# spawner1145/vae-tagger

Hardware: AMD Instinct MI355X
Metric: images/sec encode+tag, 1024^2 bf16 (higher is better)
Workload: dtype bf16

## Files before the change

vae_tagger_amd/csrc/capi.hip:

```cpp
#include <math.h>
#include <string.h>

#include "vt_context.h"
#include "vt_eval.h"

using namespace vt;

namespace {
__global__ void dbg_checksum_kernel(const unsigned int* __restrict__ p, long long n, unsigned long long* __restrict__ out) {
    unsigned long long acc = 0;
    for (long long i = (long long)blockIdx.x * blockDim.x + threadIdx.x; i < n; i += (long long)gridDim.x * blockDim.x) acc += (unsigned long long)p[i] * (unsigned long long)(i % 1021 + 1);
    atomicAdd(out, acc);
}
constexpr int DBG_SLOTS = 256;
}

void vt::dbg_sum(vt_context* c, const void* p, size_t bytes, hipStream_t s) {
    if (!c->dbg_on || !c->dbg || c->dbg_n >= DBG_SLOTS) return;
    hipLaunchKernelGGL(dbg_checksum_kernel, dim3(64), dim3(256), 0, s, (const unsigned int*)p, (long long)(bytes / 4), c->dbg + c->dbg_n);
    ++c->dbg_n;
}

extern "C" {

// ... 125 lines not shown
            d.bn_shift = (const float*)c->upload(sh.data(), H * 4);
            d.bn_w = (const float*)c->upload(g->v.data(), H * 4);
            d.bn_b = (const float*)c->upload(b->v.data(), H * 4);
            d.bn_mean = (const float*)c->upload(m->v.data(), H * 4);
            d.bn_var = (const float*)c->upload(v->v.data(), H * 4);
            if (!d.bn_scale || !d.bn_shift || !d.bn_w || !d.bn_b || !d.bn_mean || !d.bn_var) return c->fail(VT_ERR_HIP, "upload failed for batch norm");
        }
        if (d.use_self) {
            const char* p = "self_attention_post.";
            std::string s(p);
            G((s + "norm.weight").c_str(), H, &d.sa.ln_w); G((s + "norm.bias").c_str(), H, &d.sa.ln_b);
            G((s + "q_proj.weight").c_str(), H * H, &d.sa.q_w); G((s + "q_proj.bias").c_str(), H, &d.sa.q_b);
            G((s + "k_proj.weight").c_str(), H * H, &d.sa.k_w); G((s + "k_proj.bias").c_str(), H, &d.sa.k_b);
            G((s + "v_proj.weight").c_str(), H * H, &d.sa.v_w); G((s + "v_proj.bias").c_str(), H, &d.sa.v_b);
            G((s + "out_proj.weight").c_str(), H * H, &d.sa.o_w); G((s + "out_proj.bias").c_str(), H, &d.sa.o_b);
        }
        if (d.use_cross) {
            G("query_generator.weight", (int64_t)512 * H * 64, &d.qg_w); G("query_generator.bias", 512, &d.qg_b);
            G("cross_attention.q_proj.weight", 256 * 512, &d.cx_q_w); G("cross_attention.q_proj.bias", 256, &d.cx_q_b);
            G("cross_attention.k_proj.weight", 256 * H, &d.cx_k_w); G("cross_attention.k_proj.bias", 256, &d.cx_k_b);
            G("cross_attention.v_proj.weight", 256 * H, &d.cx_v_w); G("cross_attention.v_proj.bias", 256, &d.cx_v_b);
            G("cross_attention.out_proj.weight", 512 * 256, &d.cx_o_w); G("cross_attention.out_proj.bias", 512, &d.cx_o_b);
        }
        const int dims[4] = {H * 64, 1024, 512, 256};
        for (int i = 0; i < 3; ++i) {
            char k[64];
            snprintf(k, sizeof k, "classifier.%d.weight", 4 * i); G(k, (int64_t)dims[i + 1] * dims[i], &d.cls_w[i]);
            snprintf(k, sizeof k, "classifier.%d.bias", 4 * i); G(k, dims[i + 1], &d.cls_b[i]);
            snprintf(k, sizeof k, "classifier.%d.weight", 4 * i + 1); G(k, dims[i + 1], &d.cls_ln_w[i]);
            snprintf(k, sizeof k, "classifier.%d.bias", 4 * i + 1); G(k, dims[i + 1], &d.cls_ln_b[i]);
        }
        G("classifier.12.weight", (int64_t)N * 256, &d.cls_w[3]);
        G("classifier.12.bias", N, &d.cls_b[3]);
    }
#undef G
    for (auto it = c->weights.begin(); it != c->weights.end();)
        it = (it->first.compare(0, 8, "encoder.") != 0 && it->first.compare(0, 8, "decoder.") != 0) ? c->weights.erase(it) : ++it;
    c->dec_finalized = true;
    return VT_OK;
}

size_t vt_decode_workspace_bytes(const vt_context* c, int B, int h, int w) {
    if (!c || !c->dec_configured || B <= 0 || h <= 0 || w <= 0) return 0;
    return align_up(vt_decoder_workspace_floats(B, c->dec.latent_channels, h, w) * 4);
}

int vt_decode_logits(vt_context* c, const float* latent, int B, int h, int w, float* logits, void* ws, size_t ws_bytes,
                     void* stream) {
    if (!c) return VT_ERR_INVALID;
    DeviceGuard guard(c);
    if (!c->dec_finalized) return c->fail(VT_ERR_STATE, "decoder weights not finalized");
    if (!latent || !logits || !ws || B <= 0 || h <= 0 || w <= 0) return c->fail(VT_ERR_INVALID, "vt_decode_logits: bad argument");
    if (ws_bytes < vt_decode_workspace_bytes(c, B, h, w)) return c->fail(VT_ERR_WORKSPACE, "vt_decode_logits: workspace too small");
    HIPCK(c, vt_decoder_forward(c->dec, latent, B, h, w, (float*)ws, logits, (hipStream_t)stream), "decoder_forward");
    return VT_OK;
}

int vt_get_confidence(vt_context* c, const float* logits, int B, int N, float* conf, int64_t* idx, void* stream) {
    if (!c) return VT_ERR_INVALID;
    DeviceGuard guard(c);
    if (!logits || !conf || !idx || B <= 0 || N <= 0) return c->fail(VT_ERR_INVALID, "vt_get_confidence: bad argument");
    HIPCK(c, vt_decoder_sort(logits, B, N, conf, (long long*)idx, (hipStream_t)stream), "decoder_sort");
    return VT_OK;
}

int vt_summarize_confidence(vt_context* c, const float* conf, const int64_t* idx, int B, int N, float threshold, int K,
                            float* top_conf, int32_t* top_idx, float* stats, void* stream) {
    if (!c) return VT_ERR_INVALID;
    DeviceGuard guard(c);
    if (!conf || !idx || !top_conf || !top_idx || !stats || B <= 0 || N <= 0 || K <= 0) return c->fail(VT_ERR_INVALID, "vt_summarize_confidence: bad argument");
    HIPCK(c, vt_decoder_summary(conf, (const long long*)idx, B, N, threshold, K, top_conf, (int*)top_idx, stats, (hipStream_t)stream), "decoder_summary");
    return VT_OK;
}

int vt_summarize_confidence_per_class(vt_context* c, const float* conf, const int64_t* idx, int B, int N, const float* class_thresholds,
                                      int K, float* top_conf, int32_t* top_idx, float* stats, void* stream) {
    if (!c) return VT_ERR_INVALID;
    DeviceGuard guard(c);
    if (!conf || !idx || !class_thresholds || !top_conf || !top_idx || !stats || B <= 0 || N <= 0 || K <= 0)
        return c->fail(VT_ERR_INVALID, "vt_summarize_confidence_per_class: bad argument");
    HIPCK(c, vt_decoder_summary_per_class(conf, (const long long*)idx, B, N, class_thresholds, K, top_conf, (int*)top_idx, stats,
                                          (hipStream_t)stream), "decoder_summary_per_class");
    return VT_OK;
}

int vt_status(vt_context* c, int clear, int* status_out, void* stream) {
    if (!c) return VT_ERR_INVALID;
    DeviceGuard guard(c);
    if (!status_out) return c->fail(VT_ERR_INVALID, "vt_status: null output");
    hipStream_t s = (hipStream_t)stream;
    int v = 0;
    HIPCK(c, hipMemcpyAsync(&v, c->status, sizeof(int), hipMemcpyDeviceToHost, s), "vt_status copy");
    const hipError_t ec = clear ? hipMemsetAsync(c->status, 0, sizeof(int), s) : hipSuccess;
    HIPCK(c, hipStreamSynchronize(s), "vt_status sync");
    HIPCK(c, ec, "vt_status clear");
    *status_out = v;
    return VT_OK;
}

int vt_status_async(vt_context* c, int clear, int* status_out, void* stream) {
    if (!c) return VT_ERR_INVALID;
    DeviceGuard guard(c);
    if (!status_out) return c->fail(VT_ERR_INVALID, "vt_status_async: null output");
    hipStream_t s = (hipStream_t)stream;
    HIPCK(c, hipMemcpyAsync(status_out, c->status, sizeof(int), hipMemcpyDefault, s), "vt_status_async copy");
    if (clear) HIPCK(c, hipMemsetAsync(c->status, 0, sizeof(int), s), "vt_status_async clear");
    return VT_OK;
// ... 162 lines not shown

int vt_eval_merge(vt_context* c, void* dst, size_t dst_bytes, int N, int T, long long dst_capacity, long long dst_n_seen,
                  const vt_eval_source* sources, int W, void* stream) {
    if (!c) return VT_ERR_INVALID;
    DeviceGuard guard(c);
    if (int r = eval_check_state(c, "vt_eval_merge (dst)", dst, dst_bytes, N, T, dst_capacity)) return r;
    if (!sources || W < 1 || W > VT_EVAL_MAX_MERGE) return c->fail(VT_ERR_INVALID, "vt_eval_merge: null sources or W = %d outside [1, %d]", W, VT_EVAL_MAX_MERGE);
    if (dst_n_seen < 0 || dst_n_seen > VT_EVAL_MAX_N_SEEN || (dst_capacity > 0 && dst_n_seen > dst_capacity))
        return c->fail(VT_ERR_INVALID, "vt_eval_merge: dst_n_seen = %lld outside [0, capacity = %lld]", dst_n_seen, dst_capacity);
    const EvalLayout l = vt_eval_layout(N, T, dst_capacity);
    EvalMergeArg a;
    a.W = W;
    long long total = dst_n_seen;
    for (int w = 0; w < W; ++w) {
        const vt_eval_source& s = sources[w];
        if (int r = eval_check_state(c, "vt_eval_merge (source)", s.state, s.state_bytes, N, T, s.capacity)) return r;
        if (s.n_seen < 0 || s.n_seen > VT_EVAL_MAX_N_SEEN || (s.capacity > 0 && s.n_seen > s.capacity))
            return c->fail(VT_ERR_INVALID, "vt_eval_merge: source %d has n_seen = %lld outside [0, capacity = %lld]", w, s.n_seen, s.capacity);
        if (blocks_overlap(dst, l.total, s.state, vt_eval_layout(N, T, s.capacity).total))
            return c->fail(VT_ERR_INVALID, "vt_eval_merge: source %d is dst or overlaps it", w);
        if (dst_capacity > 0 && s.capacity == 0 && s.n_seen > 0)
            return c->fail(VT_ERR_INVALID, "vt_eval_merge: source %d keeps no keys (capacity 0) for its %lld samples, dst does", w, s.n_seen);
        a.src[w] = EvalMergeSrc{(const char*)s.state, s.capacity, s.n_seen, s.n_seen, total};
        total += s.n_seen;
        if (total > VT_EVAL_MAX_N_SEEN) return c->fail(VT_ERR_INVALID, "vt_eval_merge: %lld samples in all, 2^31 or more", total);
    }
    if (dst_capacity > 0 && total > dst_capacity)
        return c->fail(VT_ERR_INVALID, "vt_eval_merge: dst_n_seen + the sources' samples = %lld exceeds the capacity %lld", total, dst_capacity);
    HIPCK(c, vt_eval_launch_merge(dst, l, N, dst_capacity, a, c->eval_merge_vec, (hipStream_t)stream), "eval_merge");
    return VT_OK;
}

int vt_set_flag(vt_context* c, int flag, int value) {
    if (!c) return VT_ERR_INVALID;
    if (flag == 0) { c->use_halo_conv = value != 0; return VT_OK; }
    if (flag == 1) { c->fuse_gn_stats = value != 0; return VT_OK; }
    if (flag == 2) { c->fuse_gn_apply = value != 0; return VT_OK; }
    if (flag == 3) { c->halo_occ2 = value < 0 ? 0 : (value > 4 ? 4 : value); return VT_OK; }
    if (flag == 4) { c->res_fp16 = value != 0; return VT_OK; }
    if (flag == 5) { c->conv_in_mfma = value != 0; return VT_OK; }
    if (flag == 6) { c->gemm_short = value != 0; return VT_OK; }
    if (flag == 8) { c->fuse_shortcut = value != 0; return VT_OK; }
    if (flag == 9) { c->attn_qk_kernel = value != 0; return VT_OK; }
    if (flag == 10) { c->pv_stream = value != 0; return VT_OK; }
    if (flag == 11) { c->fp8 = value != 0; return VT_OK; }
    if (flag == 16) { if ((value & 3) == 3 || value < 0 || value > 7) return c->fail(VT_ERR_INVALID, "vt_set_flag(16): tile shape 0..2 (+4: every layer)"); c->fp8_tile = value; return VT_OK; }
    if (flag == 12) { c->attn_pv_kernel = value != 0; return VT_OK; }
    if (flag == 17) { c->attn_proj_kernel = value != 0; return VT_OK; }
    if (flag == 18) { c->f16_ops = value != 0; return VT_OK; }
    if (flag == 19) { c->s2_planar = value != 0; return VT_OK; }
    if (flag == 21) { c->eval_merge_vec = value != 0; return VT_OK; }
    if (flag == 20) { c->conv_out_halo = value != 0; return VT_OK; }
    if (flag == 22) { c->up2_literal = value != 0; return VT_OK; }
    if (flag == 13) { c->s2_halo = value != 0; return VT_OK; }
    if (flag == 14) { c->attn_fp8 = value != 0; return VT_OK; }
    if (flag == 15) { c->proj_fp8 = value != 0; return VT_OK; }
    if (flag == 7) {
        if (value < 0 || value > 2) return c->fail(VT_ERR_INVALID, "vt_set_flag(7): value %d not in 0..2", value);
        c->attn_mode = value;
        return VT_OK;
    }
    return c->fail(VT_ERR_INVALID, "vt_set_flag: unknown flag %d", flag);
}

int vt_profile_num_configs(void) { return VT_NUM_PROF_SLOTS; }

int vt_preprocess_u8(vt_context* c, const uint8_t* in_hwc, int B, int H, int W, float* out_nchw, void* stream) {
    if (!c) return VT_ERR_INVALID;
    DeviceGuard guard(c);
    HIPCK(c, vt_launch_preprocess_u8(in_hwc, out_nchw, B, H, W, (hipStream_t)stream), "vt_preprocess_u8");
    return VT_OK;
}

namespace {
constexpr int RS_BITS = 32 - 8 - 2;
double rs_filter(int kind, double x) {
    if (kind == 0) {
        if (x < 0.0) x = -x;
        return x < 1.0 ? 1.0 - x : 0.0;
    }
    if (-3.0 <= x && x < 3.0) {
        auto sinc = [](double v) { if (v == 0.0) return 1.0; v *= M_PI; return sin(v) / v; };
        return sinc(x) * sinc(x / 3);
    }
    return 0.0;
}
}
extern "C++" {
namespace vt {
int rs_ksize(int in_size, int out_size, int kind) {
    double fs = (double)in_size / out_size;
    if (fs < 1.0) fs = 1.0;
    return (int)ceil((kind == 0 ? 1.0 : 3.0) * fs) * 2 + 1;
}
void rs_table(int in_size, int out_size, int kind, int* tab) {
    const double scale = (double)in_size / out_size;
    double filterscale = scale < 1.0 ? 1.0 : scale;
    const double support = (kind == 0 ? 1.0 : 3.0) * filterscale, ss = 1.0 / filterscale;
    const int ksize = (int)ceil(support) * 2 + 1;
    std::vector<double> w(ksize);
    for (int xx = 0; xx < out_size; ++xx) {
        const double center = (xx + 0.5) * scale;
        int xmin = (int)(center - support + 0.5);
        if (xmin < 0) xmin = 0;
        int xmax = (int)(center + support + 0.5);
        if (xmax > in_size) xmax = in_size;
// ... 119 lines not shown
```

vae_tagger_amd/csrc/decoder.hip:

```cpp
#include "vt_common.h"
#include "vt_decoder.h"
#include "vt_sort_network.h"

namespace {

__global__ __launch_bounds__(256) void dec_pool_kernel(const float* __restrict__ x, int HW, float* __restrict__ pool) {
    __shared__ float red[4];
    const int c = blockIdx.x, b = blockIdx.y, C = gridDim.x;
    const float* xp = x + ((long long)b * C + c) * HW;
    float s = 0.f, m = -INFINITY;
    for (int i = threadIdx.x; i < HW; i += 256) { const float v = xp[i]; s += v; m = fmaxf(m, v); }
    s = block_sum_256(s, red);
    m = block_max_256(m, red);
    if (threadIdx.x == 0) { pool[(b * C + c) * 2] = s / (float)HW; pool[(b * C + c) * 2 + 1] = m; }
}

__global__ void dec_gate_kernel(const float* __restrict__ pool, const float* __restrict__ w0,
                                const float* __restrict__ w2, int C, int R, float* __restrict__ gate) {
    const int b = blockIdx.x, c = threadIdx.x;
    if (c >= C) return;
    float out = 0.f;
    for (int which = 0; which < 2; ++which) {
        for (int r = 0; r < R; ++r) {
            float h = 0.f;
            for (int i = 0; i < C; ++i) h = fmaf(w0[r * C + i], pool[(b * C + i) * 2 + which], h);
            h = fmaxf(h, 0.f);
            out = fmaf(w2[c * R + r], h, out);
        }
    }
    gate[b * C + c] = vt_sigmoid_accurate(out);
}

__global__ __launch_bounds__(256) void dec_spmap_kernel(const float* __restrict__ x, const float* __restrict__ gate,
                                                        int C, int HW, float* __restrict__ sp) {
    const int b = blockIdx.y;
    const int p = blockIdx.x * 256 + threadIdx.x;
    if (p >= HW) return;
    float s = 0.f, m = -INFINITY;
    for (int c = 0; c < C; ++c) {
        const float v = x[((long long)b * C + c) * HW + p] * gate[b * C + c];
        s += v; m = fmaxf(m, v);
    }
    sp[((long long)b * 2) * HW + p] = s / (float)C;
    sp[((long long)b * 2 + 1) * HW + p] = m;
}

__global__ __launch_bounds__(256) void dec_sgate_kernel(const float* __restrict__ sp, const float* __restrict__ w,
                                                        int H, int W, float* __restrict__ sg) {
    __shared__ float sw[98];
    if (threadIdx.x < 98) sw[threadIdx.x] = w[threadIdx.x];
    __syncthreads();
    const int b = blockIdx.y, HW = H * W;
    const int p = blockIdx.x * 256 + threadIdx.x;
    if (p >= HW) return;
    const int y = p / W, x = p - y * W;
    float acc = 0.f;
    for (int c = 0; c < 2; ++c)
        for (int ky = 0; ky < 7; ++ky) {
            const int iy = y + ky - 3;
            if (iy < 0 || iy >= H) continue;
            for (int kx = 0; kx < 7; ++kx) {
                const int ix = x + kx - 3;
                if (ix < 0 || ix >= W) continue;
                acc = fmaf(sw[(c * 7 + ky) * 7 + kx], sp[((long long)b * 2 + c) * HW + iy * W + ix], acc);
            }
        }
    sg[(long long)b * HW + p] = vt_sigmoid_accurate(acc);
}

template <int CO>
__global__ __launch_bounds__(256) void dec_compress_kernel(const float* __restrict__ x, const float* __restrict__ gate,
                                                           const float* __restrict__ sg, const float* __restrict__ w,
                                                           const float* __restrict__ bias,
                                                           const float* __restrict__ bn_scale,
                                                           const float* __restrict__ bn_shift, int C, int H, int W,
                                                           float* __restrict__ pooled) {
    extern __shared__ float smw[];
    __shared__ float red[4];
    __shared__ float sgate[64];
    const int cell = blockIdx.x, b = blockIdx.y, HW = H * W;
    const int cy = cell >> 3, cx = cell & 7;
    for (int i = threadIdx.x; i < CO * C * 9; i += 256) smw[i] = w[i];
    if (threadIdx.x < C) sgate[threadIdx.x] = gate ? gate[b * C + threadIdx.x] : 1.f;
    __syncthreads();
    const int y0 = (cy * H) / 8, y1 = ((cy + 1) * H + 7) / 8;
    const int x0 = (cx * W) / 8, x1 = ((cx + 1) * W + 7) / 8;
    const int ch = y1 - y0, cw = x1 - x0, n = ch * cw;
    float acc[CO];
#pragma unroll
    for (int o = 0; o < CO; ++o) acc[o] = 0.f;
    for (int i = threadIdx.x; i < n; i += 256) {
        const int y = y0 + i / cw, xx = x0 + i % cw;
        float v[CO];
#pragma unroll
        for (int o = 0; o < CO; ++o) v[o] = bias[o];
        for (int ky = 0; ky < 3; ++ky) {
            const int iy = y + ky - 1;
            if (iy < 0 || iy >= H) continue;
            for (int kx = 0; kx < 3; ++kx) {
                const int ix = xx + kx - 1;
                if (ix < 0 || ix >= W) continue;
                const int q = iy * W + ix;
                const float sgv = sg ? sg[(long long)b * HW + q] : 1.f;
                for (int c = 0; c < C; ++c) {
                    const float in = (x[((long long)b * C + c) * HW + q] * sgate[c]) * sgv;
#pragma unroll
                    for (int o = 0; o < CO; ++o) v[o] = fmaf(smw[(o * C + c) * 9 + ky * 3 + kx], in, v[o]);
                }
            }
        }
#pragma unroll
        for (int o = 0; o < CO; ++o) acc[o] += fmaxf(fmaf(v[o], bn_scale[o], bn_shift[o]), 0.f);
    }
#pragma unroll
    for (int o = 0; o < CO; ++o) {
        const float s = block_sum_256(acc[o], red);
        if (threadIdx.x == 0) pooled[((long long)b * CO + o) * 64 + cell] = s / (float)n;
    }
}

// ... 72 lines not shown
    }
#pragma unroll
    for (int o = 0; o < E; ++o) {
        float a = wts.o_b[o];
    #pragma unroll
    for (int e = 0; e < E; ++e) a = fmaf(wts.o_w[o * E + e], att[e], a);
        t[((long long)b * E + o) * 64 + tok] = a + xin[o];
    }
}

#pragma clang diagnostic pop

constexpr int LIN_BT = 8;
__global__ __launch_bounds__(256) void dec_linear_kernel(const float* __restrict__ x, const float* __restrict__ w,
                                                         const float* __restrict__ bias, float* __restrict__ y,
                                                         int B, int IN, int OUT) {
    const int lane = threadIdx.x & 63;
    const int o = blockIdx.x * 4 + (threadIdx.x >> 6);
    if (o >= OUT) return;
    const float* wr = w + (long long)o * IN;
    for (int b0 = 0; b0 < B; b0 += LIN_BT) {
        float acc[LIN_BT];
#pragma unroll
        for (int i = 0; i < LIN_BT; ++i) acc[i] = 0.f;
        for (int k = lane; k < IN; k += 64) {
            const float wv = wr[k];
#pragma unroll
            for (int i = 0; i < LIN_BT; ++i)
                if (b0 + i < B) acc[i] = fmaf(wv, x[(long long)(b0 + i) * IN + k], acc[i]);
        }
#pragma unroll
        for (int i = 0; i < LIN_BT; ++i) {
            const float s = wave_sum(acc[i]);
            if (lane == 0 && b0 + i < B) y[(long long)(b0 + i) * OUT + o] = s + bias[o];
        }
    }
}

__global__ __launch_bounds__(256) void dec_ln_act_kernel(float* __restrict__ y, const float* __restrict__ g,
                                                         const float* __restrict__ bta, int N, int act) {
    __shared__ float red[4];
    float* r = y + (long long)blockIdx.x * N;
    float s = 0.f;
    for (int i = threadIdx.x; i < N; i += 256) s += r[i];
    const float mean = block_sum_256(s, red) / (float)N;
    float v = 0.f;
    for (int i = threadIdx.x; i < N; i += 256) { const float d = r[i] - mean; v = fmaf(d, d, v); }
    const float var = block_sum_256(v, red) / (float)N;
    const float rstd = 1.0f / sqrtf(var + 1e-5f);
    for (int i = threadIdx.x; i < N; i += 256) {
        float t = (r[i] - mean) * rstd * g[i] + bta[i];
        t = act == 0 ? fmaxf(t, 0.f) : (t > 0.f ? t : 0.2f * t);
        r[i] = t;
    }
}

__global__ __launch_bounds__(256) void dec_add_rowmean_kernel(float* __restrict__ flat, const float* __restrict__ att,
                                                              int NF, int NA) {
    __shared__ float red[4];
    const int b = blockIdx.x;
    float s = 0.f;
    for (int i = threadIdx.x; i < NA; i += 256) s += att[(long long)b * NA + i];
    const float m = block_sum_256(s, red) / (float)NA;
    for (int i = threadIdx.x; i < NF; i += 256) flat[(long long)b * NF + i] += m;
}

__global__ __launch_bounds__(64) void dec_cross_attn_kernel(const float* __restrict__ qv, const float* __restrict__ feat,
                                                            const float* __restrict__ k_w, const float* __restrict__ k_b,
                                                            const float* __restrict__ v_w, const float* __restrict__ v_b,
                                                            int CH, int E, int heads, float* __restrict__ out) {
    __shared__ float so[256];
    const int b = blockIdx.x, j = threadIdx.x;
    float f[16];
    for (int c = 0; c < CH; ++c) f[c] = feat[((long long)b * CH + c) * 64 + j];
    const int hd = E / heads;
    const float scale = 1.0f / sqrtf((float)hd);
    for (int h = 0; h < heads; ++h) {
        float s = 0.f;
        for (int d = 0; d < hd; ++d) {
            const int e = h * hd + d;
            float kk = k_b[e];
            for (int c = 0; c < CH; ++c) kk = fmaf(k_w[e * CH + c], f[c], kk);
            s = fmaf(qv[(long long)b * E + e], kk, s);
        }
        s *= scale;
        const float m = wave_max(s);
        const float p = expf(s - m);
        const float den = wave_sum(p);
        for (int d = 0; d < hd; ++d) {
            const int e = h * hd + d;
            float vv = v_b[e];
            for (int c = 0; c < CH; ++c) vv = fmaf(v_w[e * CH + c], f[c], vv);
            const float o = wave_sum(p * vv) / den;
            if (j == 0) so[e] = o;
        }
    }
    __syncthreads();
    for (int e = j; e < E; e += 64) out[(long long)b * E + e] = so[e];
}

__global__ void dec_add_kernel(float* __restrict__ a, const float* __restrict__ b, long long n) {
    const long long i = (long long)blockIdx.x * blockDim.x + threadIdx.x;
    if (i < n) a[i] += b[i];
}

constexpr int SORT_CH = VT_SORT_CH;
// ... 131 lines not shown
    if (tid == 0) {
        float s5 = 0.f;
        for (int i = 0; i < 5 && i < N; ++i) s5 += c[i];
        float* o = stats + (long long)b * 4;
        o[0] = (float)base; o[1] = c[0]; o[2] = s5 / 5.0f; o[3] = (float)s_bad;
    }
}

}

#define CK(e) do { hipError_t _e = (e); if (_e != hipSuccess) return _e; } while (0)
#define CKL() CK(hipGetLastError())

DecHeadShape vt_decoder_head_shape(const DecoderWeights& w) {
    DecHeadShape h;
    const int C = w.latent_channels;
    if (w.plain) { h.hidden = 2; h.dims[0] = C * 16; h.dims[1] = 512; h.dims[2] = 256; h.dims[3] = w.num_classes; h.dims[4] = 0; h.act = 1; }
    else { h.hidden = 3; h.dims[0] = (C / 2) * 64; h.dims[1] = 1024; h.dims[2] = 512; h.dims[3] = 256; h.dims[4] = w.num_classes; h.act = 0; }
    return h;
}

hipError_t vt_dec_linear(const float* x, const float* w, const float* bias, float* y, int B, int IN, int OUT, hipStream_t s) {
    hipLaunchKernelGGL(dec_linear_kernel, dim3((OUT + 3) / 4), dim3(256), 0, s, x, w, bias, y, B, IN, OUT); CKL();
    return hipSuccess;
}
hipError_t vt_dec_ln_act(float* y, const float* g, const float* b, int rows, int N, int act, hipStream_t s) {
    hipLaunchKernelGGL(dec_ln_act_kernel, dim3(rows), dim3(256), 0, s, y, g, b, N, act); CKL();
    return hipSuccess;
}

hipError_t vt_dec_pool(const float* x, int B, int C, int HW, float* pool, hipStream_t s) {
    hipLaunchKernelGGL(dec_pool_kernel, dim3(C, B), dim3(256), 0, s, x, HW, pool); CKL();
    return hipSuccess;
}
hipError_t vt_dec_gate(const float* pool, const float* w0, const float* w2, int B, int C, int R, float* gate, hipStream_t s) {
    hipLaunchKernelGGL(dec_gate_kernel, dim3(B), dim3(64), 0, s, pool, w0, w2, C, R, gate); CKL();
    return hipSuccess;
}
hipError_t vt_dec_sgate(const float* sp, const float* w, int B, int H, int W, float* sg, hipStream_t s) {
    hipLaunchKernelGGL(dec_sgate_kernel, dim3((H * W + 255) / 256, B), dim3(256), 0, s, sp, w, H, W, sg); CKL();
    return hipSuccess;
}

hipError_t vt_dec_cross(const DecoderWeights& w, const float* x, int B, float* cq, float* cqp, float* co, float* cat, float* feat, hipStream_t s) {
    hipLaunchKernelGGL(dec_linear_kernel, dim3(512 / 4), dim3(256), 0, s, x, w.qg_w, w.qg_b, cq, B, 512, 512); CKL();
    hipLaunchKernelGGL(dec_linear_kernel, dim3(256 / 4), dim3(256), 0, s, cq, w.cx_q_w, w.cx_q_b, cqp, B, 512, 256); CKL();
    hipLaunchKernelGGL(dec_cross_attn_kernel, dim3(B), dim3(64), 0, s, cqp, x, w.cx_k_w, w.cx_k_b, w.cx_v_w, w.cx_v_b, 8, 256, w.heads, co); CKL();
    hipLaunchKernelGGL(dec_linear_kernel, dim3(512 / 4), dim3(256), 0, s, co, w.cx_o_w, w.cx_o_b, cat, B, 256, 512); CKL();
    hipLaunchKernelGGL(dec_add_kernel, dim3((B * 512 + 255) / 256), dim3(256), 0, s, cat, cq, (long long)B * 512); CKL();
    hipLaunchKernelGGL(dec_add_rowmean_kernel, dim3(B), dim3(256), 0, s, feat, cat, 512, 512); CKL();
    return hipSuccess;
}

hipError_t vt_decoder_front(const DecoderWeights& w, const float* latent, int B, int H, int Wd, float* ws, float* feat, hipStream_t s) {
    const int C = w.latent_channels, HW = H * Wd;
    if (B <= 0 || H <= 0 || Wd <= 0 || C <= 0 || C > 64) return hipErrorInvalidValue;
    if (w.plain) {
        const int n = C * 16;
        hipLaunchKernelGGL(dec_adaptive_pool_kernel, dim3((n + 255) / 256, B), dim3(256), 0, s, latent, C, H, Wd, 4, 4, feat); CKL();
        return hipSuccess;
    }
    const int CO = C / 2;
    if (CO != 8) return hipErrorInvalidValue;
    float* p = ws;
    float* pool = p; p += (size_t)B * C * 2;
    float* gate = p; p += (size_t)B * C;
    float* sp = p; p += (size_t)B * 2 * HW;
    float* sg = p; p += (size_t)B * HW;
    float* cq = p; p += (size_t)B * 512;
    float* cqp = p; p += (size_t)B * 256;
    float* co = p; p += (size_t)B * 256;
    float* cat = p; p += (size_t)B * 512;
    const float* gptr = nullptr;
    const float* sgptr = nullptr;
    if (w.use_spatial) {
        CK(vt_dec_pool(latent, B, C, HW, pool, s));
        CK(vt_dec_gate(pool, w.ca_w0, w.ca_w2, B, C, w.ca_hidden, gate, s));
        hipLaunchKernelGGL(dec_spmap_kernel, dim3((HW + 255) / 256, B), dim3(256), 0, s, latent, gate, C, HW, sp); CKL();
        CK(vt_dec_sgate(sp, w.sa_w, B, H, Wd, sg, s));
        gptr = gate; sgptr = sg;
    }
    hipLaunchKernelGGL((dec_compress_kernel<8>), dim3(64, B), dim3(256), (size_t)CO * C * 9 * sizeof(float), s, latent, gptr, sgptr,
                       w.fc_w, w.fc_b, w.bn_scale, w.bn_shift, C, H, Wd, feat); CKL();
    if (w.use_self) {
        if (CO % w.heads) return hipErrorInvalidValue;
        if (CO == 8 && w.heads == 8) hipLaunchKernelGGL((dec_self_attn_kernel<8, 8>), dim3(B), dim3(64), 0, s, feat, w.sa, CO, w.heads);
        else hipLaunchKernelGGL((dec_self_attn_kernel<0, 0>), dim3(B), dim3(64), 0, s, feat, w.sa, CO, w.heads);
        CKL();
    }
    if (w.use_cross) CK(vt_dec_cross(w, feat, B, cq, cqp, co, cat, feat, s));
    return hipSuccess;
}

hipError_t vt_decoder_head(const DecHeadShape& h, const DecHeadParams& p, const float* feat, int B, float* hbuf, float* logits, hipStream_t s) {
    const float* x = feat;
    for (int i = 0; i < h.hidden; ++i) {
        CK(vt_dec_linear(x, p.w[i], p.b[i], hbuf, B, h.dims[i], h.dims[i + 1], s));
        CK(vt_dec_ln_act(hbuf, p.ln_w[i], p.ln_b[i], B, h.dims[i + 1], h.act, s));
        x = hbuf; hbuf += (size_t)B * h.dims[i + 1];
    }
    return vt_dec_linear(x, p.w[h.hidden], p.b[h.hidden], logits, B, h.dims[h.hidden], h.dims[h.hidden + 1], s);
}

hipError_t vt_decoder_forward(const DecoderWeights& w, const float* latent, int B, int H, int Wd, float* ws,
                              float* logits, hipStream_t s) {
    const DecHeadShape h = vt_decoder_head_shape(w);
    float* feat = ws;
    float* hbuf = feat + (size_t)B * h.dims[0];
    float* front_ws = hbuf + (size_t)B * (1024 + 512 + 256);
    CK(vt_decoder_front(w, latent, B, H, Wd, front_ws, feat, s));
    DecHeadParams p;
    for (int i = 0; i < 4; ++i) { p.w[i] = w.cls_w[i]; p.b[i] = w.cls_b[i]; }
    for (int i = 0; i < 3; ++i) { p.ln_w[i] = w.cls_ln_w[i]; p.ln_b[i] = w.cls_ln_b[i]; }
    return vt_decoder_head(h, p, feat, B, hbuf, logits, s);
}

size_t vt_decoder_workspace_floats(int B, int C, int H, int Wd) {
    const size_t HW = (size_t)H * Wd;
    return (size_t)B * (C * 2 + C + 2 * HW + HW + (C / 2) * 64 + 1024 + 512 + 256 + 512 + 256 + 256 + 512 + C * 16 + 512 + 256) + 64;
}

hipError_t vt_decoder_sort(const float* logits, int B, int N, float* conf, long long* idx, hipStream_t s) {
    if (N <= 0 || B <= 0) return hipErrorInvalidValue;
    static std::atomic<unsigned long long> attr_done{0};
    CK(vt_once_per_device(attr_done, [&] {
        hipError_t e = hipFuncSetAttribute((const void*)dec_sort_local_kernel<0>, hipFuncAttributeMaxDynamicSharedMemorySize, SORT_CH * 8);
        if (e == hipSuccess) e = hipFuncSetAttribute((const void*)dec_sort_local_kernel<1>, hipFuncAttributeMaxDynamicSharedMemorySize, SORT_CH * 8);
        return e;
    }));
    const int chunks = (N + SORT_CH - 1) / SORT_CH;
    unsigned long long* keys = (unsigned long long*)idx;
    int np = 2;
    while (np < (N < SORT_CH ? N : SORT_CH)) np <<= 1;
    const size_t smem = (size_t)np * 8;
    hipLaunchKernelGGL(dec_sort_local_kernel<0>, dim3(chunks, B), dim3(1024), smem, s, logits, N, keys, conf, idx, chunks == 1 ? 1 : 0); CKL();
    if (chunks == 1) return hipSuccess;
    long long top = SORT_CH;
    while (top < N) top <<= 1;
    const unsigned pair_blocks = (unsigned)((top / 2 + 255) / 256);
    for (long long k = 2LL * SORT_CH; k <= top; k <<= 1) {
        hipLaunchKernelGGL(dec_sort_global_kernel, dim3(pair_blocks, B), dim3(256), 0, s, keys, N, (int)k, 0, 1); CKL();
        for (long long j = k >> 2; j >= SORT_CH; j >>= 1) {
            hipLaunchKernelGGL(dec_sort_global_kernel, dim3(pair_blocks, B), dim3(256), 0, s, keys, N, (int)k, (int)j, 0); CKL();
        }
        hipLaunchKernelGGL(dec_sort_local_kernel<1>, dim3(chunks, B), dim3(1024), (size_t)SORT_CH * 8, s, logits, N, keys, conf, idx, k == top ? 1 : 0); CKL();
    }
    return hipSuccess;
}

hipError_t vt_decoder_summary(const float* conf, const long long* idx, int B, int N, float threshold, int K, float* top_conf,
                              int* top_idx, float* stats, hipStream_t s) {
    if (B <= 0 || N <= 0 || K <= 0) return hipErrorInvalidValue;
    hipLaunchKernelGGL(dec_summary_kernel, dim3(B), dim3(256), 0, s, conf, idx, N, threshold, K, top_conf, top_idx, stats); CKL();
    return hipSuccess;
}

hipError_t vt_decoder_summary_per_class(const float* conf, const long long* idx, int B, int N, const float* class_thresholds, int K,
                                        float* top_conf, int* top_idx, float* stats, hipStream_t s) {
    if (B <= 0 || N <= 0 || K <= 0) return hipErrorInvalidValue;
    hipLaunchKernelGGL(dec_summary_per_class_kernel, dim3(B), dim3(256), 0, s, conf, idx, N, class_thresholds, K, top_conf, top_idx, stats); CKL();
    return hipSuccess;
}
```

vae_tagger_amd/csrc/vt_context.h:

```cpp
#pragma once
#include <hip/hip_runtime.h>
#include <stdarg.h>
#include <stdio.h>

#include <array>
#include <map>
#include <string>
#include <vector>

#include "../../include/vae_tagger_hip.h"
#include "vt_decoder.h"
#include "vt_kernels.h"

namespace vt {

struct HostTensor {
    std::vector<float> v;
    std::vector<int64_t> shape;
    int64_t numel() const { int64_t n = 1; for (auto d : shape) n *= d; return n; }
};

struct ConvW {
    const bf16_t* w = nullptr; const bf16_t* wp = nullptr; const float* b = nullptr; int cin = 0, cout = 0, k = 0;
    const bf16_t* wp2 = nullptr;
// ... 43 lines not shown
    bool has_scaling = false, has_shift = false;
    ConvW conv_in;
    int conv_in_cin() const { return (latent + 31) / 32 * 32; }
    ResnetW mid0, mid1;
    AttnW attn;
    std::vector<UpBlockW> ups;
    NormW norm_out;
    ConvW conv_out;
};

constexpr float FP8_ACT_SCALE = 8.0f;
constexpr float FP8_RES_SCALE = 1.0f;

constexpr size_t ALIGN = 256;
inline size_t align_up(size_t x) { return (x + ALIGN - 1) / ALIGN * ALIGN; }

}

struct vt_context {
    int device = 0;
    std::string err;
    std::map<std::string, vt::HostTensor> weights;
    std::vector<void*> enc_allocs, dec_allocs, imgdec_allocs;
    vt::ImageDecoderW imgdec;
    std::vector<void*>* cur_allocs = &enc_allocs;
    bool pack_fp8 = true;
    void* zeros = nullptr;
    int* status = nullptr;
    vt::EncoderW enc;
    DecoderWeights dec;
    bool dec_configured = false, dec_finalized = false;
    int use_halo_conv = 1;
    int fuse_gn_stats = 1;
    int fuse_gn_apply = 0;
    int res_fp16 = 1;
    int attn_mode = 0;
    int fuse_shortcut = 1;
    int pv_stream = 1;
    int attn_qk_kernel = 1;
    int attn_pv_kernel = 1;
    int fp8 = 0;
    int halo_occ2 = 3;
    int gemm_short = 1;
    int proj_fp8 = 1;
    int attn_fp8 = 1;
    unsigned long long* dbg = nullptr; int dbg_n = 0; bool dbg_on = false;
    int conv_out_halo = 1;
    int s2_planar = 1;
    int eval_merge_vec = 1;
    int f16_ops = 0;
    int attn_proj_kernel = 1;
    int fp8_tile = 0;
    int up2_literal = 0;
    int s2_halo = 1;
    int* rs_host = nullptr; size_t rs_host_ints = 0; hipEvent_t rs_event = nullptr;
    struct RsRingSlot { void* host = nullptr; size_t bytes = 0; hipEvent_t ev = nullptr; bool used = false; };
    static constexpr int RS_RING = 4;
    RsRingSlot rs_ring[RS_RING];
    unsigned rs_ring_next = 0;
    std::map<std::array<int, 4>, std::vector<int>> rs_tables;
    int conv_in_mfma = 1;
    void* op_scratch = nullptr; size_t op_scratch_bytes = 0;

    struct ProfRec { hipEvent_t e0, e1; double flops; int cfg; };
    bool profiling = false;
    std::vector<ProfRec> prof;
    std::vector<hipEvent_t> event_pool;
    size_t events_used = 0;
    hipEvent_t next_event() {
        if (events_used == event_pool.size()) {
            hipEvent_t e = nullptr;
            if (hipEventCreate(&e) != hipSuccess) return nullptr;
            event_pool.push_back(e);
        }
        return event_pool[events_used++];
    }

    int fail(int code, const char* fmt, ...) {
        char buf[512];
        va_list ap; va_start(ap, fmt); vsnprintf(buf, sizeof buf, fmt, ap); va_end(ap);
        err = buf;
        return code;
    }
    int hipfail(hipError_t e, const char* what) { return fail(VT_ERR_HIP, "%s: %s", what, hipGetErrorString(e)); }

    void* upload(const void* host, size_t bytes) {
        void* d = nullptr;
        if (hipMalloc(&d, bytes ? bytes : 16) != hipSuccess) return nullptr;
        cur_allocs->push_back(d);
        if (bytes && hipMemcpy(d, host, bytes, hipMemcpyHostToDevice) != hipSuccess) return nullptr;
        return d;
    }
    void free_allocs(std::vector<void*>& v) {
        for (void* p : v) (void)hipFree(p);
        v.clear();
    }
    const vt::HostTensor* find(const std::string& k) const {
        auto it = weights.find(k);
        return it == weights.end() ? nullptr : &it->second;
    }
};

namespace vt {

struct DeviceGuard {
    int prev = -1, dev;
// ... 85 lines not shown
```

vae_tagger_amd/csrc/vt_decoder.h:

```cpp
#pragma once
#include <hip/hip_runtime.h>
#include <stddef.h>

struct DecSelfAttnW {
    const float *ln_w, *ln_b, *q_w, *q_b, *k_w, *k_b, *v_w, *v_b, *o_w, *o_b;
};

struct DecoderWeights {
    int num_classes = 0;
    int latent_channels = 16;
    int heads = 8;
    int plain = 0;
    int use_spatial = 0, use_self = 0, use_cross = 0;
    int ca_hidden = 2;
    const float *ca_w0 = nullptr, *ca_w2 = nullptr, *sa_w = nullptr;
    const float *fc_w = nullptr, *fc_b = nullptr, *bn_scale = nullptr, *bn_shift = nullptr;
    const float *bn_w = nullptr, *bn_b = nullptr, *bn_mean = nullptr, *bn_var = nullptr;
    DecSelfAttnW sa{};
    const float *qg_w = nullptr, *qg_b = nullptr;
    const float *cx_q_w = nullptr, *cx_q_b = nullptr, *cx_k_w = nullptr, *cx_k_b = nullptr;
    const float *cx_v_w = nullptr, *cx_v_b = nullptr, *cx_o_w = nullptr, *cx_o_b = nullptr;
    const float* cls_w[4] = {nullptr, nullptr, nullptr, nullptr};
    const float* cls_b[4] = {nullptr, nullptr, nullptr, nullptr};
    const float* cls_ln_w[3] = {nullptr, nullptr, nullptr};
    const float* cls_ln_b[3] = {nullptr, nullptr, nullptr};
};

struct DecHeadShape { int hidden = 0; int dims[5] = {0, 0, 0, 0, 0}; int act = 0; };
struct DecHeadParams { const float* w[4]; const float* b[4]; const float* ln_w[3]; const float* ln_b[3]; };
DecHeadShape vt_decoder_head_shape(const DecoderWeights& w);
hipError_t vt_dec_linear(const float* x, const float* w, const float* bias, float* y, int B, int IN, int OUT, hipStream_t s);
hipError_t vt_dec_ln_act(float* y, const float* g, const float* b, int rows, int N, int act, hipStream_t s);
hipError_t vt_dec_pool(const float* x, int B, int C, int HW, float* pool, hipStream_t s);
hipError_t vt_dec_gate(const float* pool, const float* w0, const float* w2, int B, int C, int R, float* gate, hipStream_t s);
hipError_t vt_dec_sgate(const float* sp, const float* w, int B, int H, int W, float* sg, hipStream_t s);
hipError_t vt_dec_cross(const DecoderWeights& w, const float* x, int B, float* cq, float* cqp, float* co, float* cat, float* feat, hipStream_t s);
hipError_t vt_decoder_front(const DecoderWeights& w, const float* latent_nchw, int B, int H, int W, float* ws, float* feat, hipStream_t s);
hipError_t vt_decoder_head(const DecHeadShape& h, const DecHeadParams& p, const float* feat, int B, float* hbuf, float* logits, hipStream_t s);
hipError_t vt_decoder_forward(const DecoderWeights& w, const float* latent_nchw, int B, int H, int W, float* ws,
                              float* logits, hipStream_t s);
size_t vt_decoder_workspace_floats(int B, int C, int H, int W);
hipError_t vt_decoder_sort(const float* logits, int B, int N, float* conf, long long* idx, hipStream_t s);
hipError_t vt_decoder_summary(const float* conf, const long long* idx, int B, int N, float threshold, int K, float* top_conf,
                              int* top_idx, float* stats, hipStream_t s);
hipError_t vt_decoder_summary_per_class(const float* conf, const long long* idx, int B, int N, const float* class_thresholds, int K,
                                        float* top_conf, int* top_idx, float* stats, hipStream_t s);
```

Baseline: 217.8.

## Fuse decoder channel/spatial gate kernels and row-batched head linears with LayerNorm

Adds a tiled kernel that computes the channel gate, the gated mean/max spatial map (with halo in shared memory) and the 7x7 spatial-gate conv in one launch, replacing three kernels and the intermediate map buffer. The classifier head now runs one kernel per layer that loads up to 16 batch rows into shared memory, applies the previous LayerNorm+activation in place and does the linear with weight reuse across rows, replacing separate linear and LN launches. This targets launch overhead and repeated weight reads in the small decoder tail. Every tile recomputes the channel-gate MLP, which adds redundant work, and the head path needs large dynamic shared memory.

After: 218.2 (median of 6 runs). About the same (+0.2%).

```diff
diff --git a/vae_tagger_amd/csrc/capi.hip b/vae_tagger_amd/csrc/capi.hip
--- a/vae_tagger_amd/csrc/capi.hip
+++ b/vae_tagger_amd/csrc/capi.hip
@@ -201,7 +201,7 @@
     if (!c->dec_finalized) return c->fail(VT_ERR_STATE, "decoder weights not finalized");
     if (!latent || !logits || !ws || B <= 0 || h <= 0 || w <= 0) return c->fail(VT_ERR_INVALID, "vt_decode_logits: bad argument");
     if (ws_bytes < vt_decode_workspace_bytes(c, B, h, w)) return c->fail(VT_ERR_WORKSPACE, "vt_decode_logits: workspace too small");
-    HIPCK(c, vt_decoder_forward(c->dec, latent, B, h, w, (float*)ws, logits, (hipStream_t)stream), "decoder_forward");
+    HIPCK(c, vt_decoder_forward(c->dec, latent, B, h, w, (float*)ws, logits, (hipStream_t)stream, c->dec_fused), "decoder_forward");
     return VT_OK;
 }
 
@@ -470,6 +470,7 @@
     if (flag == 21) { c->eval_merge_vec = value != 0; return VT_OK; }
     if (flag == 20) { c->conv_out_halo = value != 0; return VT_OK; }
     if (flag == 22) { c->up2_literal = value != 0; return VT_OK; }
+    if (flag == 23) { c->dec_fused = value != 0; return VT_OK; }
     if (flag == 13) { c->s2_halo = value != 0; return VT_OK; }
     if (flag == 14) { c->attn_fp8 = value != 0; return VT_OK; }
     if (flag == 15) { c->proj_fp8 = value != 0; return VT_OK; }
diff --git a/vae_tagger_amd/csrc/decoder.hip b/vae_tagger_amd/csrc/decoder.hip
--- a/vae_tagger_amd/csrc/decoder.hip
+++ b/vae_tagger_amd/csrc/decoder.hip
@@ -66,6 +66,62 @@
             }
         }
     sg[(long long)b * HW + p] = vt_sigmoid_accurate(acc);
+}
+
+constexpr int SPG_T = 16, SPG_H = SPG_T + 6;
+__global__ __launch_bounds__(256) void dec_spgate_kernel(const float* __restrict__ x, const float* __restrict__ pool, const float* __restrict__ w0,
+                                                         const float* __restrict__ w2, const float* __restrict__ w7, int C, int R, int H, int W,
+                                                         int tiles_x, float* __restrict__ gate, float* __restrict__ sg) {
+    __shared__ float sgt[64], sw[98], ssp[2][SPG_H][SPG_H];
+    const int b = blockIdx.y, tile = blockIdx.x, tid = threadIdx.x, HW = H * W;
+    const int ty0 = (tile / tiles_x) * SPG_T, tx0 = (tile % tiles_x) * SPG_T;
+    if (tid < 98) sw[tid] = w7[tid];
+    if (tid < C) {
+        const int c = tid;
+        float out = 0.f;
+        for (int which = 0; which < 2; ++which) {
+            for (int r = 0; r < R; ++r) {
+                float h = 0.f;
+                for (int i = 0; i < C; ++i) h = fmaf(w0[r * C + i], pool[(b * C + i) * 2 + which], h);
+                h = fmaxf(h, 0.f);
+                out = fmaf(w2[c * R + r], h, out);
+            }
+        }
+        const float gv = vt_sigmoid_accurate(out);
+        sgt[c] = gv;
+        if (tile == 0) gate[b * C + c] = gv;
+    }
+    __syncthreads();
+    for (int i = tid; i < SPG_H * SPG_H; i += 256) {
+        const int ly = i / SPG_H, lx = i - ly * SPG_H;
+        const int y = ty0 + ly - 3, xx = tx0 + lx - 3;
+        float s = 0.f, m = -INFINITY;
+        if (y >= 0 && y < H && xx >= 0 && xx < W) {
+            const int p = y * W + xx;
+            for (int c = 0; c < C; ++c) {
+                const float v = x[((long long)b * C + c) * HW + p] * sgt[c];
+                s += v; m = fmaxf(m, v);
+            }
+        }
+        ssp[0][ly][lx] = s / (float)C;
+        ssp[1][ly][lx] = m;
+    }
+    __syncthreads();
+    const int ly = tid / SPG_T, lx = tid % SPG_T;
+    const int y = ty0 + ly, xx = tx0 + lx;
+    if (y >= H || xx >= W) return;
+    float acc = 0.f;
+    for (int c = 0; c < 2; ++c)
+        for (int ky = 0; ky < 7; ++ky) {
+            const int iy = y + ky - 3;
+            if (iy < 0 || iy >= H) continue;
+            for (int kx = 0; kx < 7; ++kx) {
+                const int ix = xx + kx - 3;
+                if (ix < 0 || ix >= W) continue;
+                acc = fmaf(sw[(c * 7 + ky) * 7 + kx], ssp[c][ly + ky][lx + kx], acc);
+            }
+        }
+    sg[(long long)b * HW + y * W + xx] = vt_sigmoid_accurate(acc);
 }
 
 template <int CO>
@@ -244,6 +300,94 @@
         float t = (r[i] - mean) * rstd * g[i] + bta[i];
         t = act == 0 ? fmaxf(t, 0.f) : (t > 0.f ? t : 0.2f * t);
         r[i] = t;
+    }
+}
+
+constexpr int LINR_B = 16, LINR_U = 8, LINR_S = 16, LINR_MAX_IN = 1024, LINR_MAX_BLOCKS = 512;
+template <bool LN>
+__global__ __launch_bounds__(256) void dec_linear_rows_kernel(const float* __restrict__ x, const float* __restrict__ g, const float* __restrict__ bta,
+                                                              int act, const float* __restrict__ w, const float* __restrict__ bias,
+                                                              float* __restrict__ y, int B, int IN, int OUT) {
+    extern __shared__ float sx[];
+    __shared__ float red[LINR_B][4];
+    const int tid = threadIdx.x, lane = tid & 63, wave = tid >> 6;
+    auto block_sums = [&](float (&v)[LINR_B]) {
+#pragma unroll
+        for (int r = 0; r < LINR_B; ++r) v[r] = wave_sum(v[r]);
+        __syncthreads();
+        if (lane == 0) {
+#pragma unroll
+            for (int r = 0; r < LINR_B; ++r) red[r][wave] = v[r];
+        }
+        __syncthreads();
+#pragma unroll
+        for (int r = 0; r < LINR_B; ++r) v[r] = (red[r][0] + red[r][1]) + (red[r][2] + red[r][3]);
+    };
+    for (int b0 = 0; b0 < B; b0 += LINR_B) {
+        const int nb = min(LINR_B, B - b0);
+        __syncthreads();
+        for (int i0 = tid; i0 < nb * IN; i0 += 256 * LINR_S) {
+            float v[LINR_S];
+#pragma unroll
+            for (int u = 0; u < LINR_S; ++u) v[u] = i0 + 256 * u < nb * IN ? x[(long long)b0 * IN + i0 + 256 * u] : 0.f;
+#pragma unroll
+            for (int u = 0; u < LINR_S; ++u)
+                if (i0 + 256 * u < nb * IN) sx[i0 + 256 * u] = v[u];
+        }
+        __syncthreads();
+        if (LN) {
+            float mean[LINR_B], rstd[LINR_B];
+#pragma unroll
+            for (int r = 0; r < LINR_B; ++r) {
+                float s = 0.f;
+                if (r < nb) for (int i = tid; i < IN; i += 256) s += sx[r * IN + i];
+                mean[r] = s;
+            }
+            block_sums(mean);
+#pragma unroll
+            for (int r = 0; r < LINR_B; ++r) {
+                mean[r] = mean[r] / (float)IN;
+                float v = 0.f;
+                if (r < nb) for (int i = tid; i < IN; i += 256) { const float d = sx[r * IN + i] - mean[r]; v = fmaf(d, d, v); }
+                rstd[r] = v;
+            }
+            block_sums(rstd);
+#pragma unroll
+            for (int r = 0; r < LINR_B; ++r) {
+                const float var = rstd[r] / (float)IN;
+                rstd[r] = 1.0f / sqrtf(var + 1e-5f);
+                if (r < nb) for (int i = tid; i < IN; i += 256) {
+                    float t = (sx[r * IN + i] - mean[r]) * rstd[r] * g[i] + bta[i];
+                    t = act == 0 ? fmaxf(t, 0.f) : (t > 0.f ? t : 0.2f * t);
+                    sx[r * IN + i] = t;
+                }
+            }
+            __syncthreads();
+        }
+        for (int o = blockIdx.x * 4 + wave; o < OUT; o += gridDim.x * 4) {
+            const float* wr = w + (long long)o * IN;
+            float acc[LINR_B];
+#pragma unroll
+            for (int i = 0; i < LINR_B; ++i) acc[i] = 0.f;
+            for (int k0 = lane; k0 < IN; k0 += 64 * LINR_U) {
+                float wv[LINR_U];
+#pragma unroll
+                for (int u = 0; u < LINR_U; ++u) wv[u] = k0 + 64 * u < IN ? wr[k0 + 64 * u] : 0.f;
+#pragma unroll
+                for (int u = 0; u < LINR_U; ++u) {
+                    const int k = k0 + 64 * u;
+                    if (k < IN) {
+#pragma unroll
+                        for (int i = 0; i < LINR_B; ++i) acc[i] = fmaf(wv[u], sx[i * IN + k], acc[i]);
+                    }
+                }
+            }
+#pragma unroll
+            for (int i = 0; i < LINR_B; ++i) {
+                const float s = wave_sum(acc[i]);
+                if (lane == 0 && i < nb) y[(long long)(b0 + i) * OUT + o] = s + bias[o];
+            }
+        }
     }
 }
 
@@ -481,7 +625,7 @@
     return hipSuccess;
 }
 
-hipError_t vt_decoder_front(const DecoderWeights& w, const float* latent, int B, int H, int Wd, float* ws, float* feat, hipStream_t s) {
+hipError_t vt_decoder_front(const DecoderWeights& w, const float* latent, int B, int H, int Wd, float* ws, float* feat, hipStream_t s, int fused) {
     const int C = w.latent_channels, HW = H * Wd;
     if (B <= 0 || H <= 0 || Wd <= 0 || C <= 0 || C > 64) return hipErrorInvalidValue;
     if (w.plain) {
@@ -504,9 +648,15 @@
     const float* sgptr = nullptr;
     if (w.use_spatial) {
         CK(vt_dec_pool(latent, B, C, HW, pool, s));
-        CK(vt_dec_gate(pool, w.ca_w0, w.ca_w2, B, C, w.ca_hidden, gate, s));
-        hipLaunchKernelGGL(dec_spmap_kernel, dim3((HW + 255) / 256, B), dim3(256), 0, s, latent, gate, C, HW, sp); CKL();
-        CK(vt_dec_sgate(sp, w.sa_w, B, H, Wd, sg, s));
+        if (fused) {
+            const int tx = (Wd + SPG_T - 1) / SPG_T, ty = (H + SPG_T - 1) / SPG_T;
+            hipLaunchKernelGGL(dec_spgate_kernel, dim3(tx * ty, B), dim3(256), 0, s, latent, pool, w.ca_w0, w.ca_w2, w.sa_w, C, w.ca_hidden, H, Wd,
+                               tx, gate, sg); CKL();
+        } else {
+            CK(vt_dec_gate(pool, w.ca_w0, w.ca_w2, B, C, w.ca_hidden, gate, s));
+            hipLaunchKernelGGL(dec_spmap_kernel, dim3((HW + 255) / 256, B), dim3(256), 0, s, latent, gate, C, HW, sp); CKL();
+            CK(vt_dec_sgate(sp, w.sa_w, B, H, Wd, sg, s));
+        }
         gptr = gate; sgptr = sg;
     }
     hipLaunchKernelGGL((dec_compress_kernel<8>), dim3(64, B), dim3(256), (size_t)CO * C * 9 * sizeof(float), s, latent, gptr, sgptr,
@@ -521,8 +671,29 @@
     return hipSuccess;
 }
 
-hipError_t vt_decoder_head(const DecHeadShape& h, const DecHeadParams& p, const float* feat, int B, float* hbuf, float* logits, hipStream_t s) {
+hipError_t vt_decoder_head(const DecHeadShape& h, const DecHeadParams& p, const float* feat, int B, float* hbuf, float* logits, hipStream_t s, int fused) {
     const float* x = feat;
+    bool rows = fused != 0;
+    for (int i = 0; i <= h.hidden; ++i) rows = rows && h.dims[i] <= LINR_MAX_IN;
+    if (rows) {
+        static std::atomic<unsigned long long> attr_done{0};
+        CK(vt_once_per_device(attr_done, [&] {
+            hipError_t e = hipFuncSetAttribute((const void*)dec_linear_rows_kernel<false>, hipFuncAttributeMaxDynamicSharedMemorySize, LINR_B * LINR_MAX_IN * 4);
+            if (e == hipSuccess) e = hipFuncSetAttribute((const void*)dec_linear_rows_kernel<true>, hipFuncAttributeMaxDynamicSharedMemorySize, LINR_B * LINR_MAX_IN * 4);
+            return e;
+        }));
+        for (int i = 0; i <= h.hidden; ++i) {
+            const int IN = h.dims[i], OUT = h.dims[i + 1];
+            float* out = i == h.hidden ? logits : hbuf;
+            const dim3 grid(std::min((OUT + 3) / 4, LINR_MAX_BLOCKS));
+            const size_t smem = (size_t)LINR_B * IN * sizeof(float);
+            if (i == 0) hipLaunchKernelGGL(dec_linear_rows_kernel<false>, grid, dim3(256), smem, s, x, nullptr, nullptr, h.act, p.w[i], p.b[i], out, B, IN, OUT);
+            else hipLaunchKernelGGL(dec_linear_rows_kernel<true>, grid, dim3(256), smem, s, x, p.ln_w[i - 1], p.ln_b[i - 1], h.act, p.w[i], p.b[i], out, B, IN, OUT);
+            CKL();
+            x = hbuf; hbuf += (size_t)B * OUT;
+        }
+        return hipSuccess;
+    }
     for (int i = 0; i < h.hidden; ++i) {
         CK(vt_dec_linear(x, p.w[i], p.b[i], hbuf, B, h.dims[i], h.dims[i + 1], s));
         CK(vt_dec_ln_act(hbuf, p.ln_w[i], p.ln_b[i], B, h.dims[i + 1], h.act, s));
@@ -532,16 +703,16 @@
 }
 
 hipError_t vt_decoder_forward(const DecoderWeights& w, const float* latent, int B, int H, int Wd, float* ws,
-                              float* logits, hipStream_t s) {
+                              float* logits, hipStream_t s, int fused) {
     const DecHeadShape h = vt_decoder_head_shape(w);
     float* feat = ws;
     float* hbuf = feat + (size_t)B * h.dims[0];
     float* front_ws = hbuf + (size_t)B * (1024 + 512 + 256);
-    CK(vt_decoder_front(w, latent, B, H, Wd, front_ws, feat, s));
+    CK(vt_decoder_front(w, latent, B, H, Wd, front_ws, feat, s, fused));
     DecHeadParams p;
     for (int i = 0; i < 4; ++i) { p.w[i] = w.cls_w[i]; p.b[i] = w.cls_b[i]; }
     for (int i = 0; i < 3; ++i) { p.ln_w[i] = w.cls_ln_w[i]; p.ln_b[i] = w.cls_ln_b[i]; }
-    return vt_decoder_head(h, p, feat, B, hbuf, logits, s);
+    return vt_decoder_head(h, p, feat, B, hbuf, logits, s, fused);
 }
 
 size_t vt_decoder_workspace_floats(int B, int C, int H, int Wd) {
diff --git a/vae_tagger_amd/csrc/vt_context.h b/vae_tagger_amd/csrc/vt_context.h
--- a/vae_tagger_amd/csrc/vt_context.h
+++ b/vae_tagger_amd/csrc/vt_context.h
@@ -119,6 +119,7 @@
     int attn_proj_kernel = 1;
     int fp8_tile = 0;
     int up2_literal = 0;
+    int dec_fused = 1;
     int s2_halo = 1;
     int* rs_host = nullptr; size_t rs_host_ints = 0; hipEvent_t rs_event = nullptr;
     struct RsRingSlot { void* host = nullptr; size_t bytes = 0; hipEvent_t ev = nullptr; bool used = false; };
diff --git a/vae_tagger_amd/csrc/vt_decoder.h b/vae_tagger_amd/csrc/vt_decoder.h
--- a/vae_tagger_amd/csrc/vt_decoder.h
+++ b/vae_tagger_amd/csrc/vt_decoder.h
@@ -35,10 +35,10 @@
 hipError_t vt_dec_gate(const float* pool, const float* w0, const float* w2, int B, int C, int R, float* gate, hipStream_t s);
 hipError_t vt_dec_sgate(const float* sp, const float* w, int B, int H, int W, float* sg, hipStream_t s);
 hipError_t vt_dec_cross(const DecoderWeights& w, const float* x, int B, float* cq, float* cqp, float* co, float* cat, float* feat, hipStream_t s);
-hipError_t vt_decoder_front(const DecoderWeights& w, const float* latent_nchw, int B, int H, int W, float* ws, float* feat, hipStream_t s);
-hipError_t vt_decoder_head(const DecHeadShape& h, const DecHeadParams& p, const float* feat, int B, float* hbuf, float* logits, hipStream_t s);
+hipError_t vt_decoder_front(const DecoderWeights& w, const float* latent_nchw, int B, int H, int W, float* ws, float* feat, hipStream_t s, int fused = 1);
+hipError_t vt_decoder_head(const DecHeadShape& h, const DecHeadParams& p, const float* feat, int B, float* hbuf, float* logits, hipStream_t s, int fused = 1);
 hipError_t vt_decoder_forward(const DecoderWeights& w, const float* latent_nchw, int B, int H, int W, float* ws,
-                              float* logits, hipStream_t s);
+                              float* logits, hipStream_t s, int fused = 1);
 size_t vt_decoder_workspace_floats(int B, int C, int H, int W);
 hipError_t vt_decoder_sort(const float* logits, int B, int N, float* conf, long long* idx, hipStream_t s);
 hipError_t vt_decoder_summary(const float* conf, const long long* idx, int B, int N, float threshold, int K, float* top_conf,
```
